# nschloe/flow

Measured on AMD Instinct MI355X. Metric: ipcs_time_steps_per_sec, higher is better.
Workload: dtype f64

## Files before the change

### flow_amd/_hip.py

```python
import ctypes
import os

import torch

from . import device

_HERE = os.path.dirname(os.path.abspath(__file__))
LIB_PATH = os.path.join(_HERE, 'csrc', 'libflow_hip.so')

REDUCE_WORK = 4096
MULTI_DOT_BLOCKS = 1024
GMRES_MAX_RESTART = 30
GMRES_PARTIALS = (GMRES_MAX_RESTART + 2) * 1024
GMRES_STATE = 1280
SPMV_ROWS_PER_BLOCK = 256
SPMV_NNZ_PER_BLOCK = 1022
PMG_NNZ_PER_BLOCK = 2044

c_double_p = ctypes.c_void_p
c_int_p = ctypes.c_void_p


class Operator(ctypes.Structure):
    _fields_ = [
# ... 450 lines not shown
    'flow_isoline_emit': [_P(MeshS), _P(SpaceS), _VP, _P(IsolineLevels), _VP,
                          _VP, _I, _VP, _VP, _VP, _VP, _VP, _VP],
    'flow_isoline_measure': [_P(MeshS), _P(SpaceS), _VP, _P(IsolineLevels),
                             _VP, _VP, _VP],
    'flow_region_init': [_P(SpaceS), _VP, _D, _I, _VP, _VP],
    'flow_region_sweeps': [_P(MeshS), _P(SpaceS), _I, _VP, _VP, _VP, _VP],
    'flow_region_moments': [_P(MeshS), _P(SpaceS), _VP, _D, _VP, _P(SpaceS), _I,
                            _VP, _VP, _VP, _VP],
    'flow_region_segment_sum': [_I, _VP, _VP, _I, _I, _VP, _VP, _VP],
    'flow_region_segment_minmax': [_I, _VP, _VP, _I, _I, _VP, _VP, _VP, _VP],
    'flow_multi_dot': [_I, _I, _VP, ctypes.c_size_t, _VP, _VP, _VP, _VP],
    'flow_combine': [_I, _I, _VP, ctypes.c_size_t, _I, _VP, _VP, _VP,
                     ctypes.c_size_t, _VP],
    'flow_operator_apply_block': [_P(Operator), _I, _VP, ctypes.c_size_t, _VP,
                                  ctypes.c_size_t, _VP],
    'flow_operator_apply_block_chunk': [_P(Operator), _I, _VP, ctypes.c_size_t,
                                        _VP, ctypes.c_size_t, _I, _VP],
    'flow_block_gram': [_I, _I, _VP, ctypes.c_size_t, _I, _VP, ctypes.c_size_t,
                        _VP, _VP, _VP],
    'flow_stats_update': [_I, _I, _I, _P(StatsFreq), _D, _D, _D, _VP, _VP,
                          ctypes.c_size_t, _VP],
    'flow_stats_merge': [_I, _I, _I, _I, _D, _D, _VP, _VP, ctypes.c_size_t,
                         _VP],
    }

_LIB = None


class HipError(RuntimeError):
    pass


class NotConverged(RuntimeError):
    '''Krylov / Newton non-convergence.  A RuntimeError, because callers of the
    reference catch exactly that (tests/test_boussinesq.py:254).'''


ABI_VERSION = 30


def load_library():
    global _LIB
    if _LIB is None:
        if not os.path.isfile(LIB_PATH):
            raise HipError(
                'libflow_hip.so not found at %s -- build it with '
# ... 138 lines not shown
```

### flow_amd/csrc/assembly_kernels.hip

```cpp
#include <cstdlib>

#include "fem_device.h"

namespace flow {

template <int NP>
__global__ __launch_bounds__(kBlock) void gather_kernel(
    int nout, const int* __restrict__ ptr, const int* __restrict__ src,
    const double* __restrict__ scratch, size_t plane_stride, size_t out_stride,
    double* __restrict__ out, const double* __restrict__ stop,
    const unsigned char* __restrict__ idrow = nullptr, size_t id_stride = 0,
    const double* __restrict__ v = nullptr, size_t v_stride = 0) {
  if (stopped(stop)) return;
  for (int k = blockIdx.x * blockDim.x + threadIdx.x; k < nout;
       k += gridDim.x * blockDim.x) {
    const int a = ptr[k];
    const int b = ptr[k + 1];
    double s[NP];
#pragma unroll
    for (int p = 0; p < NP; ++p) s[p] = 0.0;
    for (int t = a; t < b; t += 4) {
      int idx[4];
#pragma unroll
      for (int j = 0; j < 4; ++j) idx[j] = t + j < b ? src[t + j] : -1;
      double w[NP][4];
#pragma unroll
      for (int p = 0; p < NP; ++p)
#pragma unroll
        for (int j = 0; j < 4; ++j)
          w[p][j] = idx[j] >= 0 ? scratch[p * plane_stride + idx[j]] : 0.0;
#pragma unroll
      for (int p = 0; p < NP; ++p)
#pragma unroll
        for (int j = 0; j < 4; ++j) s[p] += w[p][j];
    }
    if (idrow) {
#pragma unroll
      for (int p = 0; p < NP; ++p)
        if (idrow[p * id_stride + k]) s[p] = v[p * v_stride + k];
    }
#pragma unroll
    for (int p = 0; p < NP; ++p) out[static_cast<size_t>(p) * out_stride + k] = s[p];
  }
}

int gather(int nout, int nplanes, const int* ptr, const int* src,
           const double* scratch, size_t plane_stride, double* out,
           hipStream_t st, size_t out_stride, int r0, int r1, const double* stop,
           const unsigned char* idrow, const double* v, size_t v_stride) {
  const size_t os = out_stride ? out_stride : static_cast<size_t>(nout);
  const size_t ids = static_cast<size_t>(nout);
  if (r1 > 0) {
    ptr += r0;
    out += r0;
    if (idrow) idrow += r0;
    if (v) v += r0;
    nout = r1 - r0;
  }
  const dim3 grid(grid_for(nout, kBlock, 1 << 20));
  FLOW_REQUIRE(nplanes == 1 || nplanes == 2, "gather: 1 or 2 planes");
  if (nplanes == 1)
    hipLaunchKernelGGL(gather_kernel<1>, grid, dim3(kBlock), 0, st, nout, ptr,
                       src, scratch, plane_stride, os, out, stop, idrow, ids, v,
                       v_stride);
  else
// ... 1148 lines not shown
  FLOW_REQUIRE(J->W->vptr && J->W->vsrc, "vector map");
  FLOW_REQUIRE(J->bfmask && J->ui && J->scratch, "matrix-free Jacobian pointers");
  FLOW_REQUIRE(J->prm.dt > 0.0 && J->prm.rho > 0.0 && J->prm.mu > 0.0,
               "parameters");
  FLOW_REQUIRE(J->nbc >= 0 && (J->nbc == 0 || J->bc_dofs), "Dirichlet dofs");
  return FLOW_OK;
}

__global__ void jvp_params_kernel(flow_ns_params prm, double* __restrict__ dst) {
  if (threadIdx.x == 0) {
    store_scalar(dst, -prm.dt / prm.rho * prm.theta_i);
    store_scalar(dst + 1, 0.5 * prm.rho);
    store_scalar(dst + 2, prm.mu);
  }
}

int flow::momentum_jvp_params(const flow_momentum_jvp* J, double* dst,
                              hipStream_t st) {
  hipLaunchKernelGGL(jvp_params_kernel, dim3(1), dim3(64), 0, st, J->prm, dst);
  FLOW_CHECK_LAUNCH();
  return FLOW_OK;
}

int flow::momentum_jvp_apply(const flow_momentum_jvp* J, const double* v,
                             double* out, hipStream_t st, int v_stride,
                             int out_stride, const double* stop,
                             const double* prm_dev) {
  const flow_mesh* mesh = J->mesh;
  const flow_space* W = J->W;
  const int nl = W->deg == 1 ? 3 : 6;
  const int vs = v_stride ? v_stride : W->n;
  const int os = out_stride ? out_stride : W->n;
  const CellRange cr(mesh);
  int rc;
  static const bool pair = [] {
    const char* e = getenv("FLOW_AMD_JVP_PAIR");
    return e && e[0] == '1';
  }();
  if (W->deg == 2 && pair) {
    hipLaunchKernelGGL(momentum_jvp_pair_kernel<2>, cell_grid(2 * cr.count()),
                       dim3(kBlock), 0, st, mesh->nc, cr.cb, cr.ce, mesh->xy,
                       W->cell_dofs, W->n, vs, J->bfmask, J->ui, v, J->prm,
                       prm_dev, J->scratch, stop);
    FLOW_CHECK_LAUNCH();
  } else {
    FLOW_DISPATCH_DEG(W->deg, momentum_jvp_kernel, cell_grid(cr.count()), st,
                      mesh->nc, cr.cb, cr.ce, mesh->xy, W->cell_dofs, W->n, vs,
                      J->bfmask, J->ui, v, J->prm, prm_dev, J->scratch, stop);
  }
  if ((rc = gather(W->n, 2, W->vptr, W->vsrc, J->scratch,
                   static_cast<size_t>(nl) * mesh->nc, out, st, os, W->r0,
                   W->r1, stop, J->nbc > 0 ? J->bc_mask : nullptr, v, vs)))
    return rc;
  if (J->nbc > 0 && !J->bc_mask) {
    const int r0 = W->r1 > 0 ? W->r0 : 0, r1 = W->r1 > 0 ? W->r1 : W->n;
    hipLaunchKernelGGL(bc_copy_kernel, dim3(grid_for(J->nbc)), dim3(kBlock), 0,
                       st, J->nbc, J->bc_dofs, W->n, r0, r1, v, vs, out, os, stop);
    FLOW_CHECK_LAUNCH();
  }
  return FLOW_OK;
}

extern "C" int flow_momentum_jvp_apply(const flow_momentum_jvp* J,
                                       const double* v, double* out,
                                       void* stream) {
  int rc = momentum_jvp_check(J);
  if (rc) return rc;
  FLOW_REQUIRE(v && out && v != out, "jvp vectors");
  return momentum_jvp_apply(J, v, out, as_stream(stream), 0, 0, nullptr);
}

// ... 188 lines not shown
```

### flow_amd/csrc/common.h

```cpp
#pragma once
#include <hip/hip_runtime.h>

#include <algorithm>
#include <cstdarg>
#include <cstdio>
#include <functional>
#include <vector>

#include "../../include/flow_hip.h"

namespace flow {
extern unsigned long long g_launches;
}
#undef hipLaunchKernelGGL
#define hipLaunchKernelGGL(kernelName, numBlocks, numThreads, memPerBlock,        \
                           streamId, ...)                                       \
  do {                                                                          \
    ++flow::g_launches;                                                         \
    (kernelName)<<<(numBlocks), (numThreads), (memPerBlock), (streamId)>>>(     \
        __VA_ARGS__);                                                           \
  } while (0)

namespace flow {

void set_error(const char* fmt, ...);

inline hipStream_t as_stream(void* s) { return static_cast<hipStream_t>(s); }

int ilu_apply(const flow_ilu* ilu, const double* in, double* out, double* work,
              hipStream_t st, const double* stop = nullptr);
int ilu_check(const flow_ilu* ilu, int op_size);

int pmg_apply(const flow_pmg* M, const double* r, double* z, hipStream_t st,
              const double* stop = nullptr);
int pmg_check(const flow_pmg* M, int op_size);
int tl_apply(const flow_tl* T, const double* r, double* z, hipStream_t st,
             const double* stop = nullptr);
int tl_check(const flow_tl* T, int op_size);
int operator_apply(const flow_operator* A, const double* x, double* y,
                   hipStream_t st, const double* stop = nullptr);
int operator_size(const flow_operator* A);
int sum_partials_host(double* work, int nparts, double* host, hipStream_t st);
int check_operator(const flow_operator* A);
int fill(int n, double value, double* y, hipStream_t st);
struct NoEarly {
  __device__ __forceinline__ void operator()(int, bool) const {}
};

enum Slot {
  kGamma = 0, kAlpha, kBeta, kRes2, kB2, kRho, kOmega, kRhoNew, kTmp,
  kBreak, kTarget2, kDone, kConvIt, kIter, kNumSlots = 16
};
int read_state(const double* S, double* host, hipStream_t st);
int check_comm(const flow_comm* c, long long need);
int check_rows(const flow_rows* R);
int exchange(const flow_comm* c, int count);
int exchange_halo(const flow_comm* C, const flow_rows* R, int ncomp, int sum_count,
                  int hoff, hipStream_t st);

int gather(int nout, int nplanes, const int* ptr, const int* src,
           const double* scratch, size_t plane_stride, double* out,
           hipStream_t st, size_t out_stride = 0, int r0 = 0, int r1 = 0,
           const double* stop = nullptr, const unsigned char* idrow = nullptr,
           const double* v = nullptr, size_t v_stride = 0);
int momentum_jvp_check(const flow_momentum_jvp* J);
int momentum_jvp_apply(const flow_momentum_jvp* J, const double* v, double* out,
                       hipStream_t st, int v_stride = 0, int out_stride = 0,
                       const double* stop = nullptr,
                       const double* prm_dev = nullptr);
int momentum_jvp_params(const flow_momentum_jvp* J, double* dst, hipStream_t st);

constexpr long long kReplayAutoRows = 1500000;
struct KeyHash {
  unsigned long long h = 1469598103934665603ull;
  void bytes(const void* p, size_t n) {
    const unsigned char* c = static_cast<const unsigned char*>(p);
    for (size_t i = 0; i < n; ++i) h = (h ^ c[i]) * 1099511628211ull;
  }
  template <class T> KeyHash& pod(const T& v) {
    bytes(&v, sizeof(T));
    return *this;
  }
  template <class T> KeyHash& obj(const T* p) {
    const unsigned char tag = p ? 1 : 0;
    bytes(&tag, 1);
    if (p) bytes(p, sizeof(T));
    return *this;
  }
};
enum ReplaySite { kReplayCg = 1, kReplayGmres = 2, kReplayMass = 4 };
bool replay_wanted(long long rows, int site);
int replay_prepare(unsigned long long key, int site, hipStream_t st,
// ... 25 lines not shown
constexpr int kBlock = 256;
constexpr int kRedBlocks = 1024;
constexpr int kMaxGrid = 2048;

inline int grid_for(long long n, int per_block = kBlock, int cap = kMaxGrid) {
  long long g = (n + per_block - 1) / per_block;
  if (g < 1) g = 1;
  if (g > cap) g = cap;
  return static_cast<int>(g);
}

__device__ __forceinline__ double load_scalar(const double* p) {
  return __hip_atomic_load(const_cast<double*>(p), __ATOMIC_RELAXED,
                           __HIP_MEMORY_SCOPE_SYSTEM);
}
__device__ __forceinline__ void store_scalar(double* p, double v) {
  __hip_atomic_store(p, v, __ATOMIC_RELAXED, __HIP_MEMORY_SCOPE_SYSTEM);
}

__device__ __forceinline__ bool stopped(const double* stop) {
  return stop != nullptr && load_scalar(stop) != 0.0;
}

constexpr int kXcdRun = 64;
__host__ __device__ __forceinline__ int xcd_tile(int b, int nwg) {
  constexpr int kGroup = 8 * kXcdRun;
  const int full = (nwg / kGroup) * kGroup;
  if (b < full) {
    const int g = b / kGroup, i = b - g * kGroup;
    return g * kGroup + (i & 7) * kXcdRun + (i >> 3);
  }
  const int nt = nwg - full, i = b - full;
  const int q = nt >> 3, r = nt & 7, xcd = i & 7;
  return full + (xcd < r ? xcd * (q + 1) : r * (q + 1) + (xcd - r) * q) +
         (i >> 3);
}

__device__ inline double block_sum(double v) {
  __shared__ double wave_part[4];
#pragma unroll
  for (int off = 32; off > 0; off >>= 1) v += __shfl_down(v, off, 64);
  const int lane = threadIdx.x & 63;
  const int wave = threadIdx.x >> 6;
  __syncthreads();
  if (lane == 0) wave_part[wave] = v;
  __syncthreads();
// ... 32 lines not shown
```

### flow_amd/csrc/la_kernels.hip

```cpp
#include <cstring>

#include "common.h"
#include "csr_stream.h"

namespace flow {

thread_local char g_error[512] = "";

void set_error(const char* fmt, ...) {
  va_list ap;
  va_start(ap, fmt);
  vsnprintf(g_error, sizeof(g_error), fmt, ap);
  va_end(ap);
}

static_assert(3 * kRedBlocks + kNumSlots <= FLOW_REDUCE_WORK, "work size");


template <bool DOT>
__global__ __launch_bounds__(kBlock) void spmv_stream_kernel(
    int n, const int* __restrict__ rowptr, const int* __restrict__ cols,
    const double* __restrict__ vals0, const double* __restrict__ vals1,
    const int* __restrict__ rowblocks, const double* __restrict__ x,
    double* __restrict__ y, double* __restrict__ dpart,
// ... 1725 lines not shown
  }
  if (nn_partial) {
    nn = block_sum(nn);
    if (threadIdx.x == 0) nn_partial[blockIdx.x] = nn;
  }
}

__global__ __launch_bounds__(kBlock) void gmres_finish_kernel(
    int nparts, int nd, const double* __restrict__ partial,
    volatile double* __restrict__ mailbox) {
  const int b = blockIdx.x;
  const int v = b < nd ? b : kGmresMax + (b - nd);
  double s = 0.0;
  for (int i = threadIdx.x; i < nparts; i += kBlock)
    s += load_scalar(partial + v * kRedBlocks + i);
  s = block_sum(s);
  if (threadIdx.x == 0) {
    mailbox[b] = s;
    __threadfence_system();
  }
}

template <int NV>
__global__ __launch_bounds__(kBlock) void gmres_combine_dev_kernel(
    int n, const double* __restrict__ coef, const double* __restrict__ cw,
    int first, const double* w, const double* __restrict__ V, size_t stride,
    double* out, double* __restrict__ nn_partial,
    const double* __restrict__ stop) {
  if (stopped(stop)) return;
  double c[NV];
#pragma unroll
  for (int k = 0; k < NV; ++k) c[k] = load_scalar(coef + k);
  const double c_w = (first && w) ? load_scalar(cw) : 0.0;
  double nn = 0.0;
  for (int i = blockIdx.x * blockDim.x + threadIdx.x; i < n;
       i += gridDim.x * blockDim.x) {
    double acc = first ? (w ? c_w * w[i] : 0.0) : out[i];
#pragma unroll
    for (int k = 0; k < NV; ++k) acc += c[k] * V[k * stride + i];
    out[i] = acc;
    nn += acc * acc;
  }
  if (nn_partial) {
    nn = block_sum(nn);
    if (threadIdx.x == 0) nn_partial[blockIdx.x] = nn;
  }
}

constexpr int kGH = 0;
constexpr int kGNrm = kGH + kGmresMax * (kGmresMax + 1);
constexpr int kGEta = kGNrm + kGmresMax + 1;
constexpr int kGCoef = kGEta + kGmresMax;
constexpr int kGCw = kGCoef + kGmresMax;
constexpr int kGYc = kGCw + 1;
constexpr int kGRot = kGYc + kGmresMax;
constexpr int kGRhs = kGRot + 2 * kGmresMax;
constexpr int kGJvp = kGRhs + kGmresMax + 1;
constexpr int kGState = kGJvp + 3;
static_assert(kGState <= FLOW_GMRES_STATE, "gmres device state");

__global__ __launch_bounds__(kBlock) void gmres_step_kernel(
    int nparts, int j, int last, double beta, double target,
    const double* __restrict__ partial, double* __restrict__ G,
    double* __restrict__ S) {
  constexpr int ld = kGmresMax + 1;
  __shared__ double val[kGmresMax + 2];
  __shared__ double Hs[kGmresMax * ld];
  __shared__ double nrm[kGmresMax + 1], eta[kGmresMax];
  __shared__ double g[kGmresMax + 1], cs[kGmresMax], sn[kGmresMax], y[kGmresMax];
// ... 184 lines not shown
                       none, cw, 1, w, V, static_cast<size_t>(N), out,
                       nn_partial);
  }
  for (int k0 = 0; k0 < nv; k0 += 8) {
    const int chunk = nv - k0 < 8 ? nv - k0 : 8;
    Coef8 coef = {};
    for (int k = 0; k < chunk; ++k) coef.c[k] = c[k0 + k];
    double* nnp = (k0 + 8 >= nv) ? nn_partial : nullptr;
#define FLOW_CALL(NV)                                                          \
  hipLaunchKernelGGL(gmres_combine_kernel<NV>, dim3(g), dim3(kBlock), 0, st, N, \
                     coef, cw, (k0 == 0 && !accumulate) ? 1 : 0, w,            \
                     V + static_cast<size_t>(k0) * N, static_cast<size_t>(N),  \
                     out, nnp)
    FLOW_NV_SWITCH(chunk, FLOW_CALL)
#undef FLOW_CALL
  }
  FLOW_CHECK_LAUNCH();
  return FLOW_OK;
}

static int gmres_combine_dev(int N, int nv, const double* coef, const double* cw,
                             const double* w, const double* V, double* out,
                             double* nn_partial, bool accumulate,
                             const double* stop, hipStream_t st) {
  const int g = grid_for(N, kBlock, kRedBlocks);
  for (int k0 = 0; k0 < nv; k0 += 8) {
    const int chunk = nv - k0 < 8 ? nv - k0 : 8;
    double* nnp = (k0 + 8 >= nv) ? nn_partial : nullptr;
#define FLOW_CALL(NV)                                                           \
  hipLaunchKernelGGL(gmres_combine_dev_kernel<NV>, dim3(g), dim3(kBlock), 0, st, \
                     N, coef + k0, cw, (k0 == 0 && !accumulate) ? 1 : 0, w,     \
                     V + static_cast<size_t>(k0) * N, static_cast<size_t>(N),   \
                     out, nnp, stop)
    FLOW_NV_SWITCH(chunk, FLOW_CALL)
#undef FLOW_CALL
  }
  FLOW_CHECK_LAUNCH();
  return FLOW_OK;
}

static double gmres_least_squares(const double (*H)[kGmresMax + 1], int j,
                                  double beta, double* y) {
  double R[kGmresMax][kGmresMax + 1];
  double g[kGmresMax + 1];
  double cs[kGmresMax], sn[kGmresMax];
  g[0] = beta;
  for (int c = 0; c < j; ++c) {
    for (int r = 0; r <= c + 1; ++r) R[c][r] = H[c][r];
    for (int i = 0; i < c; ++i) {
      const double t = cs[i] * R[c][i] + sn[i] * R[c][i + 1];
      R[c][i + 1] = -sn[i] * R[c][i] + cs[i] * R[c][i + 1];
      R[c][i] = t;
    }
    const double d = hypot(R[c][c], R[c][c + 1]);
    cs[c] = d > 0.0 ? R[c][c] / d : 1.0;
    sn[c] = d > 0.0 ? R[c][c + 1] / d : 0.0;
    R[c][c] = d;
    g[c + 1] = -sn[c] * g[c];
    g[c] = cs[c] * g[c];
  }
  for (int i = j - 1; i >= 0; --i) {
    double t = g[i];
    for (int c = i + 1; c < j; ++c) t -= R[c][i] * y[c];
    y[i] = R[i][i] != 0.0 ? t / R[i][i] : 0.0;
  }
  return fabs(g[j]);
}

static int gmres(const flow_operator* A, const double* dinv, const flow_ilu* ilu,
                 const flow_pmg* pmg, const double* b, double* x, double rtol,
                 double atol, int maxit, int m, int x_is_zero, int expected,
                 int verify, double* work, int* iters_host, double* resid_host,
                 hipStream_t st) {
  const int N = op_size(A);
  double* partial = work;
  double* S = work + 3 * kRedBlocks;
  double* V = work + FLOW_REDUCE_WORK;
  double* Z = V + static_cast<size_t>(m + 1) * N;
  double* iwork = Z + static_cast<size_t>(m) * N;
  double* P = iwork + N;
  double* Pww = P + kGmresMax * kRedBlocks;
  double* Pnn = Pww + kRedBlocks;
  double* G = P + FLOW_GMRES_PARTIALS;
  const double* stop = S + kDone;
  const int gv = grid_for(N);
  const int gd = grid_for(N, kBlock, kRedBlocks);
  int np = 0, rc;

  const double* jprm = nullptr;
  const bool precond = pmg || ilu || dinv;
  const double* Zbase = precond ? Z : V;
  auto precondition = [&](int j) -> int {
    const double* in = V + static_cast<size_t>(j) * N;
    double* out = Z + static_cast<size_t>(j) * N;
    if (pmg) return pmg_apply(pmg, in, out, st, stop);
    if (ilu) return ilu_apply(ilu, in, out, iwork, st, stop);
    if (dinv)
      hipLaunchKernelGGL(vmul_kernel, dim3(gv), dim3(kBlock), 0, st, N, 1.0, dinv,
                         in, out, stop);
    return FLOW_OK;
  };
  auto arnoldi = [&](int j, double beta, double target, bool last) -> int {
    int r;
    double* w = V + static_cast<size_t>(j + 1) * N;
    if ((r = precondition(j))) return r;
    if ((r = apply(A, Zbase + static_cast<size_t>(j) * N, w, st, nullptr, stop, 0,
                   0, jprm)))
      return r;
    for (int k0 = 0; k0 <= j; k0 += 8) {
      const int chunk = j + 1 - k0 < 8 ? j + 1 - k0 : 8;
#define FLOW_CALL(NV)                                                         \
  hipLaunchKernelGGL(gmres_dots_kernel<NV>, dim3(gd), dim3(kBlock), 0, st, N,  \
                     w, V + static_cast<size_t>(k0) * N,                      \
                     static_cast<size_t>(N), k0 == 0 ? 1 : 0,                 \
                     P + k0 * kRedBlocks, Pww, stop)
      FLOW_NV_SWITCH(chunk, FLOW_CALL)
#undef FLOW_CALL
    }
    hipLaunchKernelGGL(gmres_step_kernel, dim3(1), dim3(kBlock), 0, st, gd, j,
                       last ? 1 : 0, beta, target, P, G, S);
    FLOW_CHECK_LAUNCH();
    if (!last &&
        (r = gmres_combine_dev(N, j + 1, G + kGCoef, G + kGCw, w, V, w, Pnn, false,
                               stop, st)))
      return r;
    return FLOW_OK;
  };

  const bool replay = replay_wanted(N, kReplayGmres);
  KeyHash base;
  if (replay) {
    base.pod(0x676dull);
    key_operator(base, A, true);
    base.pod(dinv).obj(ilu).obj(ilu ? ilu->plan : nullptr).obj(pmg);
    base.pod(work).pod(N).pod(m);
    if (A->kind == 3) {
      jprm = G + kGJvp;
      if ((rc = momentum_jvp_params(
               static_cast<const flow_momentum_jvp*>(A->matfree), G + kGJvp, st)))
        return rc;
    }
  }
  auto arnoldi_replayed = [&](int j, bool last) -> int {
    if (!replay) return arnoldi(j, -1.0, 0.0, last);
    KeyHash key = base;
    key.pod(j).pod(last);
    hipGraphExec_t graph = nullptr;
// ... 242 lines not shown
                                const double* b, double* x,
                                double rtol, double atol, int maxit, int restart,
                                int x_is_zero, int expected_its, int verify,
                                double* work, size_t work_len, int* iters_host,
                                double* resid_host, void* stream) {
  int rc = check_solver_args(A, b, x, rtol, atol, maxit, 1, 0, work, work_len, 0,
                             iters_host, resid_host);
  if (rc) return rc;
  FLOW_REQUIRE(restart >= 1 && restart <= FLOW_GMRES_MAX_RESTART,
               "GMRES restart length");
  FLOW_REQUIRE(expected_its >= 0, "expected iterations");
  FLOW_REQUIRE(work_len >= FLOW_REDUCE_WORK +
                               (2 * static_cast<size_t>(restart) + 2) *
                                   op_size(A) +
                               FLOW_GMRES_PARTIALS + FLOW_GMRES_STATE,
               "solver workspace too small (FLOW_REDUCE_WORK + (2 restart + 2) N "
               "+ FLOW_GMRES_PARTIALS + FLOW_GMRES_STATE)");
  FLOW_REQUIRE(!(ilu && pmg), "one preconditioner: ilu or pmg");
  if (ilu && (rc = ilu_check(ilu, op_size(A)))) return rc;
  if (pmg && (rc = pmg_check(pmg, op_size(A)))) return rc;
  return gmres(A, dinv, ilu, pmg, b, x, rtol, atol, maxit, restart, x_is_zero,
               expected_its, verify, work, iters_host, resid_host,
               as_stream(stream));
}


namespace flow {

int check_comm(const flow_comm* c, long long need) {
  FLOW_REQUIRE(c != nullptr && c->allreduce != nullptr && c->buf != nullptr,
               "communicator");
  FLOW_REQUIRE(c->world >= 1 && c->world <= kNumSlots && c->rank >= 0 &&
                   c->rank < c->world,
               "communicator rank / world (at most 16 ranks)");
  FLOW_REQUIRE(c->capacity >= need, "exchange buffer too small");
  FLOW_REQUIRE(reinterpret_cast<uintptr_t>(c->buf) % 16 == 0,
               "exchange buffer must be 16-byte aligned");
  return FLOW_OK;
}

int check_rows(const flow_rows* R) {
  FLOW_REQUIRE(R != nullptr, "row ranges are NULL");
  FLOW_REQUIRE(0 <= R->e0 && R->e0 <= R->r0 && R->r0 < R->r1 && R->r1 <= R->e1 &&
                   R->e1 <= R->n,
               "row ranges");
  FLOW_REQUIRE(R->nhalo >= 0, "halo size");
// ... 1117 lines not shown
```

### flow_amd/csrc/pmg_kernels.hip

```cpp
#include "common.h"
#include "csr_stream16.h"

#include <hip/hip_fp16.h>

namespace flow {

__device__ __forceinline__ float2 f2(float a, float b) { return make_float2(a, b); }

template <int MODE, int FMT>
__global__ __launch_bounds__(kBlock) void pmg_cheb_kernel(
    int n, int zs, const int* __restrict__ rowptr, const void* __restrict__ cols,
    const int* __restrict__ cbase,
    const void* __restrict__ vals, const unsigned char* __restrict__ idrows,
    const int* __restrict__ rowblocks,
    const float2* __restrict__ g, const float2* rho_in, float2* rho_out,
    const float2* __restrict__ d_own, float c1, float c2,
    float2* __restrict__ d_out, float2* __restrict__ x,
    const float2* __restrict__ d_extra, double* __restrict__ z,
    const unsigned char* __restrict__ bc, const double* __restrict__ rin,
    const double* __restrict__ stop) {
  __shared__ float2 prod[kTile16];
  if (stopped(stop)) return;
  int r, r1;
  float2 s;
// ... 51 lines not shown
      acc.y += d.y;
      x[r] = acc;
    }
    return;
  }
  acc.x += own.x + d.x + extra.x;
  acc.y += own.y + d.y + extra.y;
  double zx = acc.x, zy = acc.y;
  if (bc) {
    if (bc[r]) zx = rin[r];
    if (bc[n + r]) zy = rin[static_cast<size_t>(zs) + r];
  }
  z[r] = zx;
  if (zs) z[static_cast<size_t>(zs) + r] = zy;
}

__global__ __launch_bounds__(kBlock) void pmg_init_kernel(
    int n, int rs, const double* __restrict__ r, const float2* __restrict__ dinv,
    float inv_theta, float2* __restrict__ rho0, float2* __restrict__ rho,
    float2* __restrict__ d, const double* __restrict__ stop) {
  if (stopped(stop)) return;
  for (int i = blockIdx.x * blockDim.x + threadIdx.x; i < n;
       i += gridDim.x * blockDim.x) {
    const float2 di = dinv[i];
    const float2 v = f2(static_cast<float>(r[i]) * di.x,
                        static_cast<float>(r[static_cast<size_t>(rs) + i]) * di.y);
    rho0[i] = v;
    rho[i] = v;
    d[i] = f2(inv_theta * v.x, inv_theta * v.y);
  }
}

__global__ __launch_bounds__(kBlock) void pmg_restrict_kernel(
    int n1, const int* __restrict__ rptr, const int* __restrict__ rsrc,
    const float2* __restrict__ res, const float2* __restrict__ dinv_c,
    const unsigned char* __restrict__ bcc, float inv_theta_c,
    float2* __restrict__ rhoc, float2* __restrict__ dc, float2* __restrict__ xc,
    const double* __restrict__ stop) {
  if (stopped(stop)) return;
  constexpr int kAhead = 8;
  for (int v = blockIdx.x * blockDim.x + threadIdx.x; v < n1;
       v += gridDim.x * blockDim.x) {
    const int a = rptr[v], b = rptr[v + 1];
    int idx[kAhead];
#pragma unroll
    for (int k = 0; k < kAhead; ++k) idx[k] = rsrc[a + k < b ? a + k : a];
    float2 t[kAhead];
#pragma unroll
    for (int k = 0; k < kAhead; ++k) t[k] = res[idx[k]];
    float2 s = t[0];
    float2 e = f2(0.f, 0.f);
#pragma unroll
// ... 259 lines not shown
    hipLaunchKernelGGL((pmg_cheb_kernel<MODE, 2>), dim3(L->nblocks), dim3(kBlock),
                       0, st, L->n, zs, L->rowptr, static_cast<const void*>(nullptr),
                       L->cbase, L->packed, L->idrows, L->rowblocks, g, rho_in,
                       rho_out, d_own, c1, c2, d_out, x, d_extra, z, bc, rin,
                       stop);
  else if (L->cols16)
    hipLaunchKernelGGL((pmg_cheb_kernel<MODE, 1>), dim3(L->nblocks), dim3(kBlock),
                       0, st, L->n, zs, L->rowptr,
                       static_cast<const void*>(L->cols16), L->cbase, L->vals,
                       static_cast<const unsigned char*>(nullptr), L->rowblocks,
                       g, rho_in, rho_out, d_own, c1, c2, d_out, x, d_extra, z,
                       bc, rin, stop);
  else
    hipLaunchKernelGGL((pmg_cheb_kernel<MODE, 0>), dim3(L->nblocks), dim3(kBlock),
                       0, st, L->n, zs, L->rowptr, static_cast<const void*>(L->cols),
                       L->cbase, L->vals,
                       static_cast<const unsigned char*>(nullptr), L->rowblocks,
                       g, rho_in, rho_out, d_own, c1, c2, d_out, x, d_extra, z,
                       bc, rin, stop);
}

}

int pmg_apply(const flow_pmg* M, const double* r, double* z, hipStream_t st,
              const double* stop) {
  const flow_pmg_level* F = &M->fine;
  const flow_pmg_level* C = &M->coarse;
  const int n = F->n, n1 = C->n;
  float2* w = reinterpret_cast<float2*>(M->work);
  float2* rho0 = w;
  float2* rho = rho0 + n;
  float2* d[3] = {rho + n, rho + 2 * static_cast<size_t>(n),
                  rho + 3 * static_cast<size_t>(n)};
  float2* x = rho + 4 * static_cast<size_t>(n);
  float2* crho = x + n;
  float2* cd[2] = {crho + n1, crho + 2 * static_cast<size_t>(n1)};
  float2* cx = crho + 3 * static_cast<size_t>(n1);
  const float2* fdiag = reinterpret_cast<const float2*>(F->diag);
  const float2* fdinv = reinterpret_cast<const float2*>(F->dinv);
  const float2* cdinv = reinterpret_cast<const float2*>(C->dinv);
  float2* const none = nullptr;
  double* const nod = nullptr;
  const unsigned char* const nob = nullptr;
  float c1, c2;

  Cheb pre(F->lam_min, F->lam_max);
  const int zs = M->scalar ? 0 : n;
  hipLaunchKernelGGL(pmg_init_kernel, dim3(grid_for(n)), dim3(kBlock), 0, st, n, zs,
                     r, fdinv, pre.first(), rho0, rho, d[0], stop);
  for (int j = 1; j < M->pre; ++j) {
    pre.next(&c1, &c2);
    launch_cheb<1>(F, d[j - 1], rho, rho, d[j - 1], c1, c2, d[j], none, none, nod,
                   nob, nod, stop, st);
  }
  launch_cheb<0>(F, d[M->pre - 1], rho, rho, fdiag, 0.f, 0.f, none, none, none, nod,
                 nob, nod, stop, st);
  Cheb co(C->lam_min, C->lam_max);
  hipLaunchKernelGGL(pmg_restrict_kernel, dim3(grid_for(n1)), dim3(kBlock), 0, st,
                     n1, M->rptr, M->rsrc, rho, cdinv, M->bc_coarse, co.first(),
                     crho, cd[0], cx, stop);
  for (int j = 1; j < M->coarse_steps; ++j) {
    co.next(&c1, &c2);
    float2* dn = cd[j & 1];
    const float2* dc = cd[(j - 1) & 1];
    launch_cheb<1>(C, dc, crho, crho, dc, c1, c2, dn, cx, none, nod, nob, nod,
                   stop, st);
  }
  hipLaunchKernelGGL(pmg_prolong_kernel, dim3(grid_for(n)), dim3(kBlock), 0, st, n,
                     reinterpret_cast<const int2*>(M->ends), d[0],
                     M->pre > 1 ? d[1] : none, M->pre > 2 ? d[2] : none, cx, x,
                     stop);
  Cheb post(F->lam_min, F->lam_max);
// ... 152 lines not shown
```

### include/flow_hip.h

```cpp
#ifndef FLOW_HIP_H
#define FLOW_HIP_H

#include <stddef.h>

#ifdef __cplusplus
extern "C" {
#endif

#define FLOW_OK 0
#define FLOW_NOT_CONVERGED 1
#define FLOW_INVALID 2
#define FLOW_HIP_ERROR 3

#define FLOW_SPMV_ROWS_PER_BLOCK 256
#define FLOW_SPMV_NNZ_PER_BLOCK 1022
int flow_spmv_tile_nnz(int kind);

const char* flow_last_error(void);
int flow_abi_version(void);
int flow_launch_count(unsigned long long* count_host);
int flow_graph_mode(int mode, long long auto_rows);
int flow_graph_stats(unsigned long long* stats_host);
int flow_xcd_tile_host(int block, int nblocks);

// ... 230 lines not shown
                  int* iters_host, double* resid_host, void* stream);
int flow_cg_solve_guarded(const flow_operator* A, const double* dinv,
                          const flow_coarse* coarse, const flow_mg* mg,
                          const double* b, double* x, const double* x_fallback,
                          double rtol, double atol, int maxit, int check_every,
                          int first_check, double* work, size_t work_len,
                          int* iters_host, double* resid_host,
                          int* starts_dropped_host, void* stream);
int flow_bicgstab_solve(const flow_operator* A, const double* dinv,
                        const flow_ilu* ilu, const double* b, double* x,
                        double rtol, double atol, int maxit, int check_every,
                        int first_check, double* work, size_t work_len,
                        int* iters_host, double* resid_host, void* stream);
#define FLOW_GMRES_MAX_RESTART 30
#define FLOW_GMRES_PARTIALS ((FLOW_GMRES_MAX_RESTART + 2) * 1024)
#define FLOW_GMRES_STATE 1280
int flow_gmres_solve(const flow_operator* A, const double* dinv,
                     const flow_ilu* ilu, const flow_pmg* pmg, const double* b,
                     double* x,
                     double rtol, double atol, int maxit, int restart,
                     int x_is_zero, int expected_its, int verify, double* work,
                     size_t work_len, int* iters_host, double* resid_host,
                     void* stream);

typedef int (*flow_allreduce_fn)(void* user, int count);
#define FLOW_PEER_FLAGS 16
typedef struct {
  unsigned long long* flags;
  double* land;
  int land_cap;
  int spin_limit;
  unsigned long long* nb_flags[2];
  double* nb_land[2];
  unsigned long long* seq_host;
} flow_peer;
typedef struct {
  int rank, world;
  double* buf;
  int capacity;
  flow_allreduce_fn allreduce;
  void* user;
  const flow_peer* peer;
} flow_comm;
int flow_peer_alloc(int land_cap, void** base_out, char* handle_out);
int flow_peer_open(const char* handle, void** base_out);
int flow_peer_close(void* mapped_base);
// ... 411 lines not shown
```

Measured before the change: 128.2.

## Fuse GMRES Gram-Schmidt dots into JVP gather and p-multigrid init into combine

Inside the GMRES Arnoldi step, the matrix-free momentum JVP gather kernel now also computes the dot products of its output with up to eight basis vectors and its own squared norm. It writes per-block partials that a small fold kernel reduces into the existing partial layout. Separately, the orthogonalisation combine kernel now writes the p-multigrid fine-level start vectors (rho0, rho, d0), so the next preconditioner call skips its init kernel. The intent is to avoid re-reading the new Krylov vector from memory and to save kernel launches. It adds probe entry points and an environment switch, and uses the iwork buffer as scratch for partials.

```diff
diff --git a/flow_amd/_hip.py b/flow_amd/_hip.py
--- a/flow_amd/_hip.py
+++ b/flow_amd/_hip.py
@@ -496,6 +496,10 @@
                           ctypes.c_size_t, _VP],
     'flow_stats_merge': [_I, _I, _I, _I, _D, _D, _VP, _VP, ctypes.c_size_t,
                          _VP],
+    'flow_gmres_dots_probe': [_P(Operator), _VP, _VP, _I, _I, _VP, _VP,
+                              ctypes.c_size_t, _VP, _VP],
+    'flow_gmres_combine_probe': [_I, _I, _VP, _VP, _VP, _VP, _VP, _VP,
+                                 _P(PmgS), _I, _VP],
     }
 
 _LIB = None
diff --git a/flow_amd/csrc/assembly_kernels.hip b/flow_amd/csrc/assembly_kernels.hip
--- a/flow_amd/csrc/assembly_kernels.hip
+++ b/flow_amd/csrc/assembly_kernels.hip
@@ -3,6 +3,33 @@
 #include "fem_device.h"
 
 namespace flow {
+
+template <int NP>
+__device__ __forceinline__ void gather_row(const int* __restrict__ ptr,
+                                           const int* __restrict__ src,
+                                           const double* __restrict__ scratch,
+                                           size_t plane_stride, int k,
+                                           double s[NP]) {
+  const int a = ptr[k];
+  const int b = ptr[k + 1];
+#pragma unroll
+  for (int p = 0; p < NP; ++p) s[p] = 0.0;
+  for (int t = a; t < b; t += 4) {
+    int idx[4];
+#pragma unroll
+    for (int j = 0; j < 4; ++j) idx[j] = t + j < b ? src[t + j] : -1;
+    double w[NP][4];
+#pragma unroll
+    for (int p = 0; p < NP; ++p)
+#pragma unroll
+      for (int j = 0; j < 4; ++j)
+        w[p][j] = idx[j] >= 0 ? scratch[p * plane_stride + idx[j]] : 0.0;
+#pragma unroll
+    for (int p = 0; p < NP; ++p)
+#pragma unroll
+      for (int j = 0; j < 4; ++j) s[p] += w[p][j];
+  }
+}
 
 template <int NP>
 __global__ __launch_bounds__(kBlock) void gather_kernel(
@@ -14,26 +41,8 @@
   if (stopped(stop)) return;
   for (int k = blockIdx.x * blockDim.x + threadIdx.x; k < nout;
        k += gridDim.x * blockDim.x) {
-    const int a = ptr[k];
-    const int b = ptr[k + 1];
     double s[NP];
-#pragma unroll
-    for (int p = 0; p < NP; ++p) s[p] = 0.0;
-    for (int t = a; t < b; t += 4) {
-      int idx[4];
-#pragma unroll
-      for (int j = 0; j < 4; ++j) idx[j] = t + j < b ? src[t + j] : -1;
-      double w[NP][4];
-#pragma unroll
-      for (int p = 0; p < NP; ++p)
-#pragma unroll
-        for (int j = 0; j < 4; ++j)
-          w[p][j] = idx[j] >= 0 ? scratch[p * plane_stride + idx[j]] : 0.0;
-#pragma unroll
-      for (int p = 0; p < NP; ++p)
-#pragma unroll
-        for (int j = 0; j < 4; ++j) s[p] += w[p][j];
-    }
+    gather_row<NP>(ptr, src, scratch, plane_stride, k, s);
     if (idrow) {
 #pragma unroll
       for (int p = 0; p < NP; ++p)
@@ -41,6 +50,53 @@
     }
 #pragma unroll
     for (int p = 0; p < NP; ++p) out[static_cast<size_t>(p) * out_stride + k] = s[p];
+  }
+}
+
+template <int NV>
+__global__ __launch_bounds__(kBlock) void gather_dots_kernel(
+    int nout, const int* __restrict__ ptr, const int* __restrict__ src,
+    const double* __restrict__ scratch, size_t plane_stride,
+    double* __restrict__ out, const double* __restrict__ stop,
+    const unsigned char* __restrict__ idrow, const double* __restrict__ v,
+    const double* __restrict__ V, size_t stride, double* __restrict__ part) {
+  if (stopped(stop)) return;
+  __shared__ double wave_part[NV + 1][4];
+  double acc[NV + 1];
+#pragma unroll
+  for (int c = 0; c <= NV; ++c) acc[c] = 0.0;
+  for (int k = blockIdx.x * blockDim.x + threadIdx.x; k < nout;
+       k += gridDim.x * blockDim.x) {
+    double b0[NV], b1[NV];
+#pragma unroll
+    for (int c = 0; c < NV; ++c) {
+      b0[c] = V[c * stride + k];
+      b1[c] = V[c * stride + nout + k];
+    }
+    double s[2];
+    gather_row<2>(ptr, src, scratch, plane_stride, k, s);
+    if (idrow) {
+      if (idrow[k]) s[0] = v[k];
+      if (idrow[static_cast<size_t>(nout) + k]) s[1] = v[static_cast<size_t>(nout) + k];
+    }
+    out[k] = s[0];
+    out[static_cast<size_t>(nout) + k] = s[1];
+#pragma unroll
+    for (int c = 0; c < NV; ++c) acc[c] += s[0] * b0[c] + s[1] * b1[c];
+    acc[NV] += s[0] * s[0] + s[1] * s[1];
+  }
+#pragma unroll
+  for (int c = 0; c <= NV; ++c) {
+    double a = acc[c];
+#pragma unroll
+    for (int off = 32; off > 0; off >>= 1) a += __shfl_down(a, off, 64);
+    if ((threadIdx.x & 63) == 0) wave_part[c][threadIdx.x >> 6] = a;
+  }
+  __syncthreads();
+  if (threadIdx.x <= NV) {
+    const int c = threadIdx.x;
+    part[static_cast<size_t>(c) * gridDim.x + blockIdx.x] =
+        (wave_part[c][0] + wave_part[c][1]) + (wave_part[c][2] + wave_part[c][3]);
   }
 }
 
@@ -1235,10 +1291,18 @@
   return FLOW_OK;
 }
 
+bool flow::momentum_jvp_fuses_dots(const flow_momentum_jvp* J) {
+  return J->W->r1 <= 0 && (J->nbc == 0 || J->bc_mask != nullptr);
+}
+
+int flow::gather_dots_parts(const flow_momentum_jvp* J) {
+  return grid_for(J->W->n, kBlock, 1 << 20);
+}
+
 int flow::momentum_jvp_apply(const flow_momentum_jvp* J, const double* v,
                              double* out, hipStream_t st, int v_stride,
                              int out_stride, const double* stop,
-                             const double* prm_dev) {
+                             const double* prm_dev, const GatherDots* dots) {
   const flow_mesh* mesh = J->mesh;
   const flow_space* W = J->W;
   const int nl = W->deg == 1 ? 3 : 6;
@@ -1260,6 +1324,34 @@
     FLOW_DISPATCH_DEG(W->deg, momentum_jvp_kernel, cell_grid(cr.count()), st,
                       mesh->nc, cr.cb, cr.ce, mesh->xy, W->cell_dofs, W->n, vs,
                       J->bfmask, J->ui, v, J->prm, prm_dev, J->scratch, stop);
+  }
+  if (dots) {
+    FLOW_REQUIRE(momentum_jvp_fuses_dots(J) && v_stride == 0 && out_stride == 0,
+                 "fused Gram-Schmidt dots: whole vectors, Dirichlet byte mask");
+    FLOW_REQUIRE(dots->V && dots->part && dots->nv >= 1 &&
+                     dots->nv <= kGatherDotsMax &&
+                     dots->nparts == gather_dots_parts(J),
+                 "fused Gram-Schmidt dots: operands");
+    const dim3 grid(dots->nparts);
+    const unsigned char* mask = J->nbc > 0 ? J->bc_mask : nullptr;
+#define FLOW_CALL(NV)                                                           \
+  hipLaunchKernelGGL(gather_dots_kernel<NV>, grid, dim3(kBlock), 0, st, W->n,   \
+                     W->vptr, W->vsrc, J->scratch,                             \
+                     static_cast<size_t>(nl) * mesh->nc, out, stop, mask, v,   \
+                     dots->V, dots->stride, dots->part)
+    switch (dots->nv) {
+      case 1: FLOW_CALL(1); break;
+      case 2: FLOW_CALL(2); break;
+      case 3: FLOW_CALL(3); break;
+      case 4: FLOW_CALL(4); break;
+      case 5: FLOW_CALL(5); break;
+      case 6: FLOW_CALL(6); break;
+      case 7: FLOW_CALL(7); break;
+      default: FLOW_CALL(8); break;
+    }
+#undef FLOW_CALL
+    FLOW_CHECK_LAUNCH();
+    return FLOW_OK;
   }
   if ((rc = gather(W->n, 2, W->vptr, W->vsrc, J->scratch,
                    static_cast<size_t>(nl) * mesh->nc, out, st, os, W->r0,
diff --git a/flow_amd/csrc/common.h b/flow_amd/csrc/common.h
--- a/flow_amd/csrc/common.h
+++ b/flow_amd/csrc/common.h
@@ -32,8 +32,19 @@
 int ilu_check(const flow_ilu* ilu, int op_size);
 
 int pmg_apply(const flow_pmg* M, const double* r, double* z, hipStream_t st,
-              const double* stop = nullptr);
+              const double* stop = nullptr, bool init_done = false);
 int pmg_check(const flow_pmg* M, int op_size);
+struct PmgStart {
+  int n, rs;
+  const float* dinv;
+  float inv_theta;
+  float* rho0;
+  float* rho;
+  float* d0;
+};
+PmgStart pmg_start(const flow_pmg* M);
+int pmg_init(const flow_pmg* M, const double* r, hipStream_t st,
+             const double* stop = nullptr);
 int tl_apply(const flow_tl* T, const double* r, double* z, hipStream_t st,
              const double* stop = nullptr);
 int tl_check(const flow_tl* T, int op_size);
@@ -64,10 +75,21 @@
            const double* stop = nullptr, const unsigned char* idrow = nullptr,
            const double* v = nullptr, size_t v_stride = 0);
 int momentum_jvp_check(const flow_momentum_jvp* J);
+struct GatherDots {
+  const double* V;
+  size_t stride;
+  int nv;
+  double* part;
+  int nparts;
+};
+constexpr int kGatherDotsMax = 8;
+bool momentum_jvp_fuses_dots(const flow_momentum_jvp* J);
+int gather_dots_parts(const flow_momentum_jvp* J);
 int momentum_jvp_apply(const flow_momentum_jvp* J, const double* v, double* out,
                        hipStream_t st, int v_stride = 0, int out_stride = 0,
                        const double* stop = nullptr,
-                       const double* prm_dev = nullptr);
+                       const double* prm_dev = nullptr,
+                       const GatherDots* dots = nullptr);
 int momentum_jvp_params(const flow_momentum_jvp* J, double* dst, hipStream_t st);
 
 constexpr long long kReplayAutoRows = 1500000;
@@ -139,6 +161,13 @@
   return stop != nullptr && load_scalar(stop) != 0.0;
 }
 
+__device__ __forceinline__ void pmg_start_row(double r0, double r1, float2 di,
+                                              float inv_theta, float2* v,
+                                              float2* d) {
+  *v = make_float2(static_cast<float>(r0) * di.x, static_cast<float>(r1) * di.y);
+  *d = make_float2(inv_theta * v->x, inv_theta * v->y);
+}
+
 constexpr int kXcdRun = 64;
 __host__ __device__ __forceinline__ int xcd_tile(int b, int nwg) {
   constexpr int kGroup = 8 * kXcdRun;
diff --git a/flow_amd/csrc/la_kernels.hip b/flow_amd/csrc/la_kernels.hip
--- a/flow_amd/csrc/la_kernels.hip
+++ b/flow_amd/csrc/la_kernels.hip
@@ -1,3 +1,4 @@
+#include <cstdlib>
 #include <cstring>
 
 #include "common.h"
@@ -1771,6 +1772,16 @@
 }
 
 template <int NV>
+__device__ __forceinline__ double gmres_combine_entry(
+    const double (&c)[NV], double c_w, int first, const double* w,
+    const double* __restrict__ V, size_t stride, const double* out, size_t i) {
+  double acc = first ? (w ? c_w * w[i] : 0.0) : out[i];
+#pragma unroll
+  for (int k = 0; k < NV; ++k) acc += c[k] * V[k * stride + i];
+  return acc;
+}
+
+template <int NV>
 __global__ __launch_bounds__(kBlock) void gmres_combine_dev_kernel(
     int n, const double* __restrict__ coef, const double* __restrict__ cw,
     int first, const double* w, const double* __restrict__ V, size_t stride,
@@ -1784,9 +1795,7 @@
   double nn = 0.0;
   for (int i = blockIdx.x * blockDim.x + threadIdx.x; i < n;
        i += gridDim.x * blockDim.x) {
-    double acc = first ? (w ? c_w * w[i] : 0.0) : out[i];
-#pragma unroll
-    for (int k = 0; k < NV; ++k) acc += c[k] * V[k * stride + i];
+    const double acc = gmres_combine_entry<NV>(c, c_w, first, w, V, stride, out, i);
     out[i] = acc;
     nn += acc * acc;
   }
@@ -1794,6 +1803,58 @@
     nn = block_sum(nn);
     if (threadIdx.x == 0) nn_partial[blockIdx.x] = nn;
   }
+}
+
+template <int NV>
+__global__ __launch_bounds__(kBlock) void gmres_combine_pmg_kernel(
+    int n, int rs, const double* __restrict__ coef, const double* __restrict__ cw,
+    int first, const double* w, const double* __restrict__ V, size_t stride,
+    double* out, double* __restrict__ nn_partial,
+    const double* __restrict__ stop, const float2* __restrict__ dinv,
+    float inv_theta, float2* __restrict__ rho0, float2* __restrict__ rho,
+    float2* __restrict__ d0) {
+  if (stopped(stop)) return;
+  double c[NV];
+#pragma unroll
+  for (int k = 0; k < NV; ++k) c[k] = load_scalar(coef + k);
+  const double c_w = (first && w) ? load_scalar(cw) : 0.0;
+  double nn = 0.0;
+  for (int i = blockIdx.x * blockDim.x + threadIdx.x; i < n;
+       i += gridDim.x * blockDim.x) {
+    const double a0 = gmres_combine_entry<NV>(c, c_w, first, w, V, stride, out, i);
+    out[i] = a0;
+    nn += a0 * a0;
+    double a1 = a0;
+    if (rs) {
+      const size_t i1 = static_cast<size_t>(rs) + i;
+      a1 = gmres_combine_entry<NV>(c, c_w, first, w, V, stride, out, i1);
+      out[i1] = a1;
+      nn += a1 * a1;
+    }
+    float2 v, d;
+    pmg_start_row(a0, a1, dinv[i], inv_theta, &v, &d);
+    rho0[i] = v;
+    rho[i] = v;
+    d0[i] = d;
+  }
+  if (nn_partial) {
+    nn = block_sum(nn);
+    if (threadIdx.x == 0) nn_partial[blockIdx.x] = nn;
+  }
+}
+
+__global__ __launch_bounds__(kBlock) void gmres_fold_kernel(
+    int nin, int nv, const double* __restrict__ Q, int nout,
+    double* __restrict__ P, double* __restrict__ Pww,
+    const double* __restrict__ stop) {
+  if (stopped(stop)) return;
+  const int b = blockIdx.x * blockDim.x + threadIdx.x;
+  const int c = blockIdx.y;
+  if (b >= nout) return;
+  const double* __restrict__ q = Q + static_cast<size_t>(c) * nin;
+  double s = 0.0;
+  for (int i = b; i < nin; i += nout) s += load_scalar(q + i);
+  (c < nv ? P + c * kRedBlocks : Pww)[b] = s;
 }
 
 constexpr int kGH = 0;
@@ -2024,11 +2085,29 @@
 static int gmres_combine_dev(int N, int nv, const double* coef, const double* cw,
                              const double* w, const double* V, double* out,
                              double* nn_partial, bool accumulate,
-                             const double* stop, hipStream_t st) {
+                             const double* stop, hipStream_t st,
+                             const PmgStart* start = nullptr) {
   const int g = grid_for(N, kBlock, kRedBlocks);
   for (int k0 = 0; k0 < nv; k0 += 8) {
     const int chunk = nv - k0 < 8 ? nv - k0 : 8;
     double* nnp = (k0 + 8 >= nv) ? nn_partial : nullptr;
+    if (start && k0 + 8 >= nv) {
+      FLOW_REQUIRE((start->rs ? 2 : 1) * static_cast<long long>(start->n) == N,
+                   "p-multigrid start: size");
+#define FLOW_CALL(NV)                                                           \
+  hipLaunchKernelGGL(gmres_combine_pmg_kernel<NV>, dim3(g), dim3(kBlock), 0, st, \
+                     start->n, start->rs, coef + k0, cw,                        \
+                     (k0 == 0 && !accumulate) ? 1 : 0, w,                       \
+                     V + static_cast<size_t>(k0) * N, static_cast<size_t>(N),   \
+                     out, nnp, stop,                                            \
+                     reinterpret_cast<const float2*>(start->dinv),              \
+                     start->inv_theta, reinterpret_cast<float2*>(start->rho0),  \
+                     reinterpret_cast<float2*>(start->rho),                     \
+                     reinterpret_cast<float2*>(start->d0))
+      FLOW_NV_SWITCH(chunk, FLOW_CALL)
+#undef FLOW_CALL
+      continue;
+    }
 #define FLOW_CALL(NV)                                                           \
   hipLaunchKernelGGL(gmres_combine_dev_kernel<NV>, dim3(g), dim3(kBlock), 0, st, \
                      N, coef + k0, cw, (k0 == 0 && !accumulate) ? 1 : 0, w,     \
@@ -2067,6 +2146,56 @@
     y[i] = R[i][i] != 0.0 ? t / R[i][i] : 0.0;
   }
   return fabs(g[j]);
+}
+
+static bool gmres_fused() {
+  static const bool on = [] {
+    const char* e = getenv("FLOW_AMD_GMRES_FUSED");
+    return !(e && e[0] == '0');
+  }();
+  return on;
+}
+
+static bool gmres_dots_fusable(const flow_momentum_jvp* J, int N) {
+  return momentum_jvp_fuses_dots(J) &&
+         static_cast<long long>(kGatherDotsMax + 1) * gather_dots_parts(J) <= N;
+}
+
+static int gmres_apply_dots(const flow_operator* A, const double* z, double* w,
+                            const double* V, int nd, double* P, double* Pww,
+                            double* Q, bool fused, const double* jprm,
+                            const double* stop, hipStream_t st) {
+  const int N = op_size(A);
+  const int gd = grid_for(N, kBlock, kRedBlocks);
+  int r, k0 = 0;
+  if (fused) {
+    const flow_momentum_jvp* J = static_cast<const flow_momentum_jvp*>(A->matfree);
+    GatherDots dots;
+    dots.V = V;
+    dots.stride = static_cast<size_t>(N);
+    dots.nv = nd < kGatherDotsMax ? nd : kGatherDotsMax;
+    dots.part = Q;
+    dots.nparts = gather_dots_parts(J);
+    if ((r = momentum_jvp_apply(J, z, w, st, 0, 0, stop, jprm, &dots))) return r;
+    hipLaunchKernelGGL(gmres_fold_kernel, dim3(grid_for(gd), dots.nv + 1),
+                       dim3(kBlock), 0, st, dots.nparts, dots.nv, Q, gd, P, Pww,
+                       stop);
+    k0 = dots.nv;
+  } else if ((r = apply(A, z, w, st, nullptr, stop, 0, 0, jprm))) {
+    return r;
+  }
+  for (; k0 < nd; k0 += 8) {
+    const int chunk = nd - k0 < 8 ? nd - k0 : 8;
+#define FLOW_CALL(NV)                                                         \
+  hipLaunchKernelGGL(gmres_dots_kernel<NV>, dim3(gd), dim3(kBlock), 0, st, N,  \
+                     w, V + static_cast<size_t>(k0) * N,                      \
+                     static_cast<size_t>(N), k0 == 0 ? 1 : 0,                 \
+                     P + k0 * kRedBlocks, Pww, stop)
+    FLOW_NV_SWITCH(chunk, FLOW_CALL)
+#undef FLOW_CALL
+  }
+  FLOW_CHECK_LAUNCH();
+  return FLOW_OK;
 }
 
 static int gmres(const flow_operator* A, const double* dinv, const flow_ilu* ilu,
@@ -2090,12 +2219,18 @@
   int np = 0, rc;
 
   const double* jprm = nullptr;
+  const bool fuse_dots =
+      gmres_fused() && A->kind == 3 &&
+      gmres_dots_fusable(static_cast<const flow_momentum_jvp*>(A->matfree), N);
+  const bool fuse_init = gmres_fused() && pmg != nullptr;
+  PmgStart start = {};
+  if (fuse_init) start = pmg_start(pmg);
   const bool precond = pmg || ilu || dinv;
   const double* Zbase = precond ? Z : V;
   auto precondition = [&](int j) -> int {
     const double* in = V + static_cast<size_t>(j) * N;
     double* out = Z + static_cast<size_t>(j) * N;
-    if (pmg) return pmg_apply(pmg, in, out, st, stop);
+    if (pmg) return pmg_apply(pmg, in, out, st, stop, fuse_init && j > 0);
     if (ilu) return ilu_apply(ilu, in, out, iwork, st, stop);
     if (dinv)
       hipLaunchKernelGGL(vmul_kernel, dim3(gv), dim3(kBlock), 0, st, N, 1.0, dinv,
@@ -2106,25 +2241,15 @@
     int r;
     double* w = V + static_cast<size_t>(j + 1) * N;
     if ((r = precondition(j))) return r;
-    if ((r = apply(A, Zbase + static_cast<size_t>(j) * N, w, st, nullptr, stop, 0,
-                   0, jprm)))
+    if ((r = gmres_apply_dots(A, Zbase + static_cast<size_t>(j) * N, w, V, j + 1,
+                              P, Pww, iwork, fuse_dots, jprm, stop, st)))
       return r;
-    for (int k0 = 0; k0 <= j; k0 += 8) {
-      const int chunk = j + 1 - k0 < 8 ? j + 1 - k0 : 8;
-#define FLOW_CALL(NV)                                                         \
-  hipLaunchKernelGGL(gmres_dots_kernel<NV>, dim3(gd), dim3(kBlock), 0, st, N,  \
-                     w, V + static_cast<size_t>(k0) * N,                      \
-                     static_cast<size_t>(N), k0 == 0 ? 1 : 0,                 \
-                     P + k0 * kRedBlocks, Pww, stop)
-      FLOW_NV_SWITCH(chunk, FLOW_CALL)
-#undef FLOW_CALL
-    }
     hipLaunchKernelGGL(gmres_step_kernel, dim3(1), dim3(kBlock), 0, st, gd, j,
                        last ? 1 : 0, beta, target, P, G, S);
     FLOW_CHECK_LAUNCH();
     if (!last &&
         (r = gmres_combine_dev(N, j + 1, G + kGCoef, G + kGCw, w, V, w, Pnn, false,
-                               stop, st)))
+                               stop, st, fuse_init ? &start : nullptr)))
       return r;
     return FLOW_OK;
   };
@@ -2413,6 +2538,55 @@
   return gmres(A, dinv, ilu, pmg, b, x, rtol, atol, maxit, restart, x_is_zero,
                expected_its, verify, work, iters_host, resid_host,
                as_stream(stream));
+}
+
+extern "C" int flow_gmres_dots_probe(const flow_operator* A, const double* z,
+                                     const double* V, int nd, int fused,
+                                     double* w, double* work, size_t work_len,
+                                     double* h, void* stream) {
+  int rc = check_operator(A);
+  if (rc) return rc;
+  FLOW_REQUIRE(A->kind == 3, "the matrix-free operator");
+  FLOW_REQUIRE(z && V && w && work && h, "pointers");
+  FLOW_REQUIRE(nd >= 1 && nd <= kGmresMax, "basis vectors");
+  const int N = op_size(A);
+  FLOW_REQUIRE(work_len >= FLOW_GMRES_PARTIALS + static_cast<size_t>(N),
+               "workspace (FLOW_GMRES_PARTIALS + N)");
+  FLOW_REQUIRE(!fused || gmres_dots_fusable(
+                             static_cast<const flow_momentum_jvp*>(A->matfree), N),
+               "this operator's gather cannot carry the dots");
+  hipStream_t st = as_stream(stream);
+  double* P = work;
+  double* Pww = P + kGmresMax * kRedBlocks;
+  if ((rc = gmres_apply_dots(A, z, w, V, nd, P, Pww, work + FLOW_GMRES_PARTIALS,
+                             fused != 0, nullptr, nullptr, st)))
+    return rc;
+  hipLaunchKernelGGL(gmres_finish_kernel, dim3(nd + 1), dim3(kBlock), 0, st,
+                     grid_for(N, kBlock, kRedBlocks), nd, P, h);
+  FLOW_CHECK_LAUNCH();
+  return FLOW_OK;
+}
+
+extern "C" int flow_gmres_combine_probe(int N, int nv, const double* coef,
+                                        const double* cw, const double* w,
+                                        const double* V, double* out,
+                                        double* nn_partial,
+                                        const flow_pmg* pmg, int fused,
+                                        void* stream) {
+  FLOW_REQUIRE(N > 0 && nv >= 1 && nv <= kGmresMax, "sizes");
+  FLOW_REQUIRE(coef && cw && w && V && out && nn_partial, "pointers");
+  FLOW_REQUIRE(pmg && pmg->work && pmg->fine.dinv && pmg->fine.n > 0 &&
+                   pmg->fine.lam_max > pmg->fine.lam_min && pmg->fine.lam_min > 0.0,
+               "flow_pmg (fine.n, fine.dinv, interval, work)");
+  FLOW_REQUIRE((pmg->scalar ? 1 : 2) * static_cast<long long>(pmg->fine.n) == N,
+               "flow_pmg does not match N");
+  hipStream_t st = as_stream(stream);
+  const PmgStart start = pmg_start(pmg);
+  int rc;
+  if ((rc = gmres_combine_dev(N, nv, coef, cw, w, V, out, nn_partial, false,
+                              nullptr, st, fused ? &start : nullptr)))
+    return rc;
+  return fused ? FLOW_OK : pmg_init(pmg, out, st, nullptr);
 }
 
 
diff --git a/flow_amd/csrc/pmg_kernels.hip b/flow_amd/csrc/pmg_kernels.hip
--- a/flow_amd/csrc/pmg_kernels.hip
+++ b/flow_amd/csrc/pmg_kernels.hip
@@ -97,12 +97,12 @@
   if (stopped(stop)) return;
   for (int i = blockIdx.x * blockDim.x + threadIdx.x; i < n;
        i += gridDim.x * blockDim.x) {
-    const float2 di = dinv[i];
-    const float2 v = f2(static_cast<float>(r[i]) * di.x,
-                        static_cast<float>(r[static_cast<size_t>(rs) + i]) * di.y);
+    float2 v, d0;
+    pmg_start_row(r[i], r[static_cast<size_t>(rs) + i], dinv[i], inv_theta, &v,
+                  &d0);
     rho0[i] = v;
     rho[i] = v;
-    d[i] = f2(inv_theta * v.x, inv_theta * v.y);
+    d[i] = d0;
   }
 }
 
@@ -408,8 +408,34 @@
 
 }
 
+PmgStart pmg_start(const flow_pmg* M) {
+  const int n = M->fine.n;
+  float2* w = reinterpret_cast<float2*>(M->work);
+  PmgStart s;
+  s.n = n;
+  s.rs = M->scalar ? 0 : n;
+  s.dinv = M->fine.dinv;
+  s.inv_theta = Cheb(M->fine.lam_min, M->fine.lam_max).first();
+  s.rho0 = reinterpret_cast<float*>(w);
+  s.rho = reinterpret_cast<float*>(w + n);
+  s.d0 = reinterpret_cast<float*>(w + 2 * static_cast<size_t>(n));
+  return s;
+}
+
+int pmg_init(const flow_pmg* M, const double* r, hipStream_t st,
+             const double* stop) {
+  const PmgStart s = pmg_start(M);
+  hipLaunchKernelGGL(pmg_init_kernel, dim3(grid_for(s.n)), dim3(kBlock), 0, st,
+                     s.n, s.rs, r, reinterpret_cast<const float2*>(s.dinv),
+                     s.inv_theta, reinterpret_cast<float2*>(s.rho0),
+                     reinterpret_cast<float2*>(s.rho),
+                     reinterpret_cast<float2*>(s.d0), stop);
+  FLOW_CHECK_LAUNCH();
+  return FLOW_OK;
+}
+
 int pmg_apply(const flow_pmg* M, const double* r, double* z, hipStream_t st,
-              const double* stop) {
+              const double* stop, bool init_done) {
   const flow_pmg_level* F = &M->fine;
   const flow_pmg_level* C = &M->coarse;
   const int n = F->n, n1 = C->n;
@@ -423,7 +449,6 @@
   float2* cd[2] = {crho + n1, crho + 2 * static_cast<size_t>(n1)};
   float2* cx = crho + 3 * static_cast<size_t>(n1);
   const float2* fdiag = reinterpret_cast<const float2*>(F->diag);
-  const float2* fdinv = reinterpret_cast<const float2*>(F->dinv);
   const float2* cdinv = reinterpret_cast<const float2*>(C->dinv);
   float2* const none = nullptr;
   double* const nod = nullptr;
@@ -432,8 +457,10 @@
 
   Cheb pre(F->lam_min, F->lam_max);
   const int zs = M->scalar ? 0 : n;
-  hipLaunchKernelGGL(pmg_init_kernel, dim3(grid_for(n)), dim3(kBlock), 0, st, n, zs,
-                     r, fdinv, pre.first(), rho0, rho, d[0], stop);
+  if (!init_done) {
+    const int rc = pmg_init(M, r, st, stop);
+    if (rc) return rc;
+  }
   for (int j = 1; j < M->pre; ++j) {
     pre.next(&c1, &c2);
     launch_cheb<1>(F, d[j - 1], rho, rho, d[j - 1], c1, c2, d[j], none, none, nod,
diff --git a/include/flow_hip.h b/include/flow_hip.h
--- a/include/flow_hip.h
+++ b/include/flow_hip.h
@@ -276,6 +276,14 @@
                      int x_is_zero, int expected_its, int verify, double* work,
                      size_t work_len, int* iters_host, double* resid_host,
                      void* stream);
+
+int flow_gmres_dots_probe(const flow_operator* A, const double* z,
+                          const double* V, int nd, int fused, double* w,
+                          double* work, size_t work_len, double* h, void* stream);
+int flow_gmres_combine_probe(int N, int nv, const double* coef, const double* cw,
+                             const double* w, const double* V, double* out,
+                             double* nn_partial, const flow_pmg* pmg, int fused,
+                             void* stream);
 
 typedef int (*flow_allreduce_fn)(void* user, int count);
 #define FLOW_PEER_FLAGS 16
```

Result: no change. 127.8 (-0.3%).
